# yoseph007/PQA2

Hardware: AMD Instinct MI355X
Metric: VMAF frames/sec (vif+adm+motion2 -> SVM), device-resident synthetic YUV pairs (higher is better)
Workload: dtype f32; 1 GPU; 2160p 3840x2160 8-bit, vmaf_4k_v0.6.1, 300 frames/GPU; frames_per_gpu=300, frames_total=300, batch=97, frames_per_launch=75, clips_pipelined=True, parallelism=frame-shard x1, 1-frame motion halo, all-gather of records + of scores

## Files before the change

### pqa2_amd/csrc/kernels.h

```cpp
#pragma once
#include <hip/hip_runtime.h>
#include <stdint.h>

#include <vector>

namespace pqa {

enum Elem : int { ELEM_U8 = 0, ELEM_U16 = 1, ELEM_F32 = 2 };

struct PlaneRun {
  const void* base;
  int64_t row_pitch;
  int64_t frame_pitch;
};

struct MutPlaneRun {
  void* base;
  int64_t row_pitch;
  int64_t frame_pitch;
};

int vif_tile_w(int scale);
constexpr int kVifTileH = 8;
inline int vif_tiles_x(int scale, int w) { return (w + vif_tile_w(scale) - 1) / vif_tile_w(scale); }
// ... 30 lines not shown
                      float inv_scale, float gain_limit, MutPlaneRun ll_ref, MutPlaneRun ll_dis, double* partials,
                      int* n_partials, hipError_t* err);
bool adm_pyramid_takes(Elem elem, int w, int h);
int adm_pyramid_partials(int w, int h);
bool launch_adm_pyramid(hipStream_t stream, Elem elem, PlaneRun ref, PlaneRun dis, int n_frames, int w, int h, float inv_scale,
                        float gain_limit, MutPlaneRun ll_ref, MutPlaneRun ll_dis, double* partials0, double* partials1,
                        int* n_partials, hipError_t* err);
float adm_dwt_quant_step(int lambda, int theta);

constexpr int kAdmFxRows = kAdmTileH + 2;
struct AdmFxScale {
  int scale, band_w, band_h;
  int left, top, right, bottom;
  float rf[3];
  uint32_t i_rf[3];
  int cm_shift_sq[3], cm_shift_sub[3], cm_shift_cub[3], cm_final_q[3];
  int den_shift_sq, den_shift_cub, den_final_q;
  int num_row_shift, den_row_shift;
};
AdmFxScale adm_fixed_scale_params(int scale, int band_w, int band_h);
void adm_fixed_div_table(int32_t* out65537);
void adm_fixed_epilogue(const AdmFxScale& p, const long long acc[6], double* num_out, double* den_out);
hipError_t launch_adm_fixed(hipStream_t stream, int scale, int bit_depth, Elem elem, PlaneRun ref, PlaneRun dis,
                            int n_frames, int w, int h, double gain_limit, const int32_t* div_lut,
                            MutPlaneRun ll_ref, MutPlaneRun ll_dis, long long* partials);

constexpr int kMotionTileW = 252, kMotionTileH = 16;
inline int motion_tiles(int w, int h) {
  return ((w + kMotionTileW - 1) / kMotionTileW) * ((h + kMotionTileH - 1) / kMotionTileH);
}
enum : int { MOTION_TILED = 0, MOTION_AUTO = 1 };
hipError_t launch_motion(hipStream_t stream, Elem elem, PlaneRun ref, const void* prev0, int64_t prev0_row_pitch,
                         int n_frames, int w, int h, float inv_scale, double* partials, int mode = MOTION_AUTO,
                         int* n_partials = nullptr);
int motion_march_partials(int w, int h);
bool launch_motion_march(hipStream_t stream, Elem elem, PlaneRun ref, const void* prev0, int64_t prev0_row_pitch, int n_frames,
                         int w, int h, double* partials, int* n_partials, hipError_t* err);
hipError_t launch_motion_fixed(hipStream_t stream, int bit_depth, Elem elem, PlaneRun ref, const void* prev0,
                               int64_t prev0_row_pitch, int n_frames, int w, int h, unsigned long long* partials);

constexpr int kSseBlocksPerPlane = 256;
hipError_t launch_sse(hipStream_t stream, Elem elem, PlaneRun a, PlaneRun b, int n_frames, int w, int h,
                      unsigned long long* partials);

constexpr int kSsimTileBW = 32, kSsimTileBH = 8;
inline int ssim_tiles(int w, int h) {
  const int ww = (w >> 2) - 1, wh = (h >> 2) - 1;
  if (ww < 1 || wh < 1) return 0;
  return ((ww + kSsimTileBW - 1) / kSsimTileBW) * ((wh + kSsimTileBH - 1) / kSsimTileBH);
}
hipError_t launch_ssim(hipStream_t stream, Elem elem, PlaneRun main, PlaneRun ref, int n_frames, int w, int h,
                       int max_value, double* partials, unsigned long long* sse_partials);

constexpr int kLumaBlocks = 128;
hipError_t launch_luma_stats(hipStream_t stream, Elem elem, PlaneRun luma, int n_frames, int w, int h,
                             unsigned threshold, int gray_bit_depth, unsigned long long* partials,
                             unsigned long long* out);
void luma_gray_map(int bit_depth, float* a, float* b);

struct FinalizeArgs {
  int n_frames;
  int has_vif, has_adm, has_motion, n_sse_planes, n_ssim_planes;
  const double* vif_part[4];   int vif_tiles[4];
  const long long* vif_fx_part[4];
  const double* adm_part[4];   int adm_tiles[4];   float adm_area[4];
  const long long* adm_fx_part[4];
  int adm_fx_tiles_x[4], adm_fx_top[4], adm_fx_bottom[4], adm_fx_num_shift[4], adm_fx_den_shift[4];
  long long* adm_fx_acc;
  const double* motion_part;   int motion_tiles;   double motion_norm;
  const unsigned long long* motion_fx_part;
// ... 225 lines not shown
```

### pqa2_amd/csrc/motion.hip

```cpp
#include "kernels.h"
#include "pqa_device.h"

namespace pqa {
namespace {

struct MotionArgs {
  const void* ref;
  int64_t row_pitch, frame_pitch;
  const void* prev0;
  int64_t prev0_row_pitch;
  int w, h, tiles_x, n_tiles;
  double* partials;
  f2 vt[6];
  f2 ht[5];
};

constexpr int TW = kMotionTileW, TH = kMotionTileH, R = 2, COLS = TW + 4, NSEG = TW / 4, S = 16, NIN = S + 4;
constexpr int kP2 = 258;
static_assert(COLS <= 256 && NSEG <= 64 && TW % 4 == 0 && TH == S, "one column per thread, one 16-row strip");

template <typename T>
__global__ __launch_bounds__(kBlock) void motion_kernel(const MotionArgs a) {
  __shared__ f2 sv[TH / 2][kP2];
  __shared__ double red[4];
// ... 54 lines not shown
    if (seg < NSEG) {
      f2 in[8];
      const f4* p = reinterpret_cast<const f4*>(&sv[rp][seg * 4]);
#pragma unroll
      for (int q = 0; q < 4; ++q) {
        const f4 v = p[q];
        in[2 * q] = f2{v.x, v.y};
        in[2 * q + 1] = f2{v.z, v.w};
      }
      f2 out[4];
#pragma unroll
      for (int o = 0; o < 4; ++o) out[o] = f2{0.0f, 0.0f};
#pragma unroll
      for (int k = 0; k < 5; ++k)
#pragma unroll
        for (int o = 0; o < 4; ++o) out[o] = __builtin_elementwise_fma(a.ht[k], in[o + k], out[o]);
#pragma unroll
      for (int o = 0; o < 4; ++o) {
        const float mc = (x0 + seg * 4 + o) < a.w ? 1.0f : 0.0f;
        sad = fmaf(mc * mA, fabsf(out[o].x), sad);
        sad = fmaf(mc * mB, fabsf(out[o].y), sad);
      }
    }
  }
  const float part[1] = {sad};
  double v[1];
  block_sum_f32<1>(part, v, red);
  if (tid == 0) a.partials[(int64_t)fr * a.n_tiles + tile] = v[0];
}

}

hipError_t launch_motion(hipStream_t stream, Elem elem, PlaneRun ref, const void* prev0, int64_t prev0_row_pitch,
                         int n_frames, int w, int h, float inv_scale, double* partials, int mode, int* n_partials) {
  if (n_partials) *n_partials = motion_tiles(w, h);
  if (n_frames <= 0) return hipSuccess;
  if (mode == MOTION_AUTO) {
    hipError_t err = hipSuccess;
    if (launch_motion_march(stream, elem, ref, prev0, prev0_row_pitch, n_frames, w, h, partials, n_partials, &err)) return err;
  }
  MotionArgs a{};
  a.ref = ref.base; a.row_pitch = ref.row_pitch; a.frame_pitch = ref.frame_pitch;
  a.prev0 = prev0; a.prev0_row_pitch = prev0_row_pitch;
  a.w = w; a.h = h;
  a.tiles_x = (w + TW - 1) / TW;
  a.n_tiles = motion_tiles(w, h);
  (void)inv_scale;
  a.partials = partials;
  {
    double v[5], sum = 0.0;
    float f[5];
    for (int k = 0; k < 5; ++k) { v[k] = exp(-0.5 * (k - 2) * (k - 2)); sum += v[k]; }
    for (int k = 0; k < 5; ++k) f[k] = (float)(v[k] / sum);
    for (int k = 0; k <= 5; ++k) a.vt[k] = f2{k < 5 ? f[k] : 0.0f, k > 0 ? f[k - 1] : 0.0f};
    for (int k = 0; k < 5; ++k) a.ht[k] = f2{f[k], f[k]};
  }
  const dim3 grid(a.n_tiles, n_frames), block(kBlock);
  switch (elem) {
    case ELEM_U8: hipLaunchKernelGGL((motion_kernel<uint8_t>), grid, block, 0, stream, a); break;
    case ELEM_U16: hipLaunchKernelGGL((motion_kernel<uint16_t>), grid, block, 0, stream, a); break;
    default: return hipErrorInvalidValue;
  }
  return hipGetLastError();
}

}
```

### pqa2_amd/csrc/motion_march.hip

```cpp
#include <cmath>

#include "kernels.h"
#include "pqa_device.h"

namespace pqa {
namespace {

constexpr int kCols = 124;

struct MotionMarchArgs {
  const void* ref;
  unsigned pitch;
  int64_t frame_pitch;
  const void* prev0;
  unsigned prev0_pitch;
  int w, h;
  int aligned, aligned0;
  int n_stripes, n_sg, seg_rows, n_seg;
  float c[5];
  double* partials;
  int n_part;
};

__device__ __forceinline__ float from_left(float v) {
  return __builtin_bit_cast(float, __builtin_amdgcn_update_dpp(0, __builtin_bit_cast(int, v), 0x138, 0xf, 0xf, true));
}
__device__ __forceinline__ float from_right(float v) {
  return __builtin_bit_cast(float, __builtin_amdgcn_update_dpp(0, __builtin_bit_cast(int, v), 0x130, 0xf, 0xf, true));
}

template <typename T, bool EDGE>
struct PairLoader {
  rsrc_t rs;
  unsigned v0, v1, pitch;
  int h;
  struct Raw { unsigned a, b; };
  __device__ __forceinline__ Raw load(int y) const {
    const unsigned so = (unsigned)mirror1(y, h) * pitch;
    if constexpr (EDGE) {
      return Raw{(unsigned)buf_load<T>(rs, v0, so), (unsigned)buf_load<T>(rs, v1, so)};
    } else if constexpr (sizeof(T) == 1) {
      return Raw{(unsigned)(unsigned short)__builtin_amdgcn_raw_buffer_load_b16(rs, v0, so, 0), 0u};
    } else {
      return Raw{(unsigned)__builtin_amdgcn_raw_buffer_load_b32(rs, v0 * 2u, so * 2u, 0), 0u};
    }
  }
  static __device__ __forceinline__ f2 to_float(const Raw r) {
    if constexpr (EDGE) return f2{(float)r.a, (float)r.b};
    else if constexpr (sizeof(T) == 1) return f2{(float)(r.a & 0xffu), (float)((r.a >> 8) & 0xffu)};
    else return f2{(float)(r.a & 0xffffu), (float)(r.a >> 16)};
  }
};

template <typename T, bool EDGE>
__device__ __forceinline__ double march(const MotionMarchArgs& a, const PairLoader<T, EDGE>& cur, const PairLoader<T, EDGE>& prv,
                                        const int r0, const int r1, const int x_first ) {
  const float c0 = a.c[0], c1 = a.c[1], c2 = a.c[2], c3 = a.c[3], c4 = a.c[4];
  f2 p0 = f2{0.0f, 0.0f}, p1 = p0, p2 = p0, p3 = p0;
  float sad0 = 0.0f, sad1 = 0.0f;
  double dsad0 = 0.0, dsad1 = 0.0;
  const int y_end = min(r1, a.h);
  typename PairLoader<T, EDGE>::Raw cs[4], ps[4];
#pragma unroll
  for (int j = 0; j < 4; ++j) { cs[j] = cur.load(r0 - 2 + j); ps[j] = prv.load(r0 - 2 + j); }
  int step = 0;
  for (int y = r0 - 2; y < r1 + 2; y += 4, ++step) {
    f2 d[4];
#pragma unroll
    for (int j = 0; j < 4; ++j) d[j] = PairLoader<T, EDGE>::to_float(cs[j]) - PairLoader<T, EDGE>::to_float(ps[j]);
#pragma unroll
    for (int j = 0; j < 4; ++j) { cs[j] = cur.load(y + 4 + j); ps[j] = prv.load(y + 4 + j); }
    const f2 k0 = f2{c0, c0}, k1 = f2{c1, c1}, k2 = f2{c2, c2}, k3 = f2{c3, c3}, k4 = f2{c4, c4};
    f2 o[4];
    o[0] = __builtin_elementwise_fma(k4, d[0], p0);
    o[1] = __builtin_elementwise_fma(k4, d[1], __builtin_elementwise_fma(k3, d[0], p1));
    o[2] = __builtin_elementwise_fma(k4, d[2], __builtin_elementwise_fma(k3, d[1], __builtin_elementwise_fma(k2, d[0], p2)));
    o[3] = __builtin_elementwise_fma(k4, d[3], __builtin_elementwise_fma(k3, d[2], __builtin_elementwise_fma(k2, d[1], __builtin_elementwise_fma(k1, d[0], p3))));
    p0 = __builtin_elementwise_fma(k3, d[3], __builtin_elementwise_fma(k2, d[2], __builtin_elementwise_fma(k1, d[1], k0 * d[0])));
    p1 = __builtin_elementwise_fma(k2, d[3], __builtin_elementwise_fma(k1, d[2], k0 * d[1]));
    p2 = __builtin_elementwise_fma(k1, d[3], k0 * d[2]);
    p3 = k0 * d[3];
#pragma unroll
    for (int j = 0; j < 4; ++j) {
      const int yo = y - 2 + j;
      const float wrow = __builtin_bit_cast(float, (unsigned)-(int)(yo >= r0 && yo < y_end) & 0x3f800000u);
      const float m0 = o[j].x, m1 = o[j].y;
      const float l0 = from_left(m0), l1 = from_left(m1), q0 = from_right(m0), q1 = from_right(m1);
      const float h0 = fmaf(c4, q0, fmaf(c3, m1, fmaf(c2, m0, fmaf(c1, l1, c0 * l0))));
      const float h1 = fmaf(c4, q1, fmaf(c3, q0, fmaf(c2, m1, fmaf(c1, m0, c0 * l1))));
      sad0 = fmaf(wrow, fabsf(h0), sad0);
      sad1 = fmaf(wrow, fabsf(h1), sad1);
    }
    if ((step & 3) == 3) { dsad0 += (double)sad0; dsad1 += (double)sad1; sad0 = 0.0f; sad1 = 0.0f; }
  }
  dsad0 += (double)sad0;
  dsad1 += (double)sad1;
  const int lane = threadIdx.x & 63;
  const bool own = lane >= 1 && lane <= 62;
  return (own && x_first < a.w ? dsad0 : 0.0) + (own && x_first + 1 < a.w ? dsad1 : 0.0);
}

#ifndef PQA_MOTION_SEG_ROWS
#define PQA_MOTION_SEG_ROWS 128
#endif

template <typename T>
__global__ __launch_bounds__(kBlock) void motion_march_kernel(const MotionMarchArgs a) {
  const int tid = threadIdx.x, lane = tid & 63;
  const int wave = __builtin_amdgcn_readfirstlane(tid >> 6);
  const int id = xcd_remap(blockIdx.x, a.n_sg * a.n_seg);
  const int sg = id % a.n_sg, seg = id / a.n_sg;
  const int stripe = sg * 4 + wave;
  const int fr = blockIdx.y;
  double* __restrict__ part = a.partials + (int64_t)fr * a.n_part + (int64_t)id * 4 + wave;
  const T* __restrict__ cur = (const T*)a.ref + (int64_t)fr * a.frame_pitch;
  const T* __restrict__ prev = fr == 0 ? (const T*)a.prev0 : cur - a.frame_pitch;
  const unsigned pitch_p = fr == 0 ? a.prev0_pitch : a.pitch;
  if (stripe >= a.n_stripes || prev == nullptr) {
    if (lane == 0) *part = 0.0;
    return;
  }
  const int r0 = seg * a.seg_rows, r1 = min(r0 + a.seg_rows, a.h);
  const int cs = stripe * (kCols / 2);
  const int c = cs - 1 + lane;
  const rsrc_t rs_c = make_rsrc(cur, (unsigned)a.h * a.pitch * (unsigned)sizeof(T));
  const rsrc_t rs_p = make_rsrc(prev, (unsigned)a.h * pitch_p * (unsigned)sizeof(T));
  const bool fast = a.aligned && (fr > 0 || a.aligned0) && cs >= 1 && 2 * (cs + kCols / 2) + 1 < a.w;
  double v;
  if (fast) {
    const PairLoader<T, false> lc{rs_c, (unsigned)(2 * c), 0u, a.pitch, a.h}, lp{rs_p, (unsigned)(2 * c), 0u, pitch_p, a.h};
    v = march<T, false>(a, lc, lp, r0, r1, 2 * c);
  } else {
    const unsigned v0 = (unsigned)mirror1(2 * c, a.w), v1 = (unsigned)mirror1(2 * c + 1, a.w);
    const PairLoader<T, true> lc{rs_c, v0, v1, a.pitch, a.h}, lp{rs_p, v0, v1, pitch_p, a.h};
    v = march<T, true>(a, lc, lp, r0, r1, 2 * c);
  }
  v = wave_sum(v);
  if (lane == 0) *part = v;
}

}

int motion_march_partials(int w, int h) {
  const int n_stripes = (w + kCols - 1) / kCols;
  return ((n_stripes + 3) / 4) * 4 * ((h + PQA_MOTION_SEG_ROWS - 1) / PQA_MOTION_SEG_ROWS);
}

bool launch_motion_march(hipStream_t stream, Elem elem, PlaneRun ref, const void* prev0, int64_t prev0_row_pitch, int n_frames,
                         int w, int h, double* partials, int* n_partials, hipError_t* err) {
  if (elem != ELEM_U8 && elem != ELEM_U16) return false;
  const int es = elem == ELEM_U16 ? 2 : 1;
  if ((int64_t)ref.row_pitch * h * es >= (1ll << 31) || (int64_t)prev0_row_pitch * h * es >= (1ll << 31)) return false;
  MotionMarchArgs a{};
  a.ref = ref.base; a.pitch = (unsigned)ref.row_pitch; a.frame_pitch = ref.frame_pitch;
  a.prev0 = prev0; a.prev0_pitch = (unsigned)prev0_row_pitch;
  a.w = w; a.h = h;
  const uintptr_t two = (uintptr_t)(2 * es - 1);
  a.aligned = ((uintptr_t)ref.base & two) == 0 && ((ref.row_pitch | ref.frame_pitch) & 1) == 0;
  a.aligned0 = ((uintptr_t)prev0 & two) == 0 && (prev0_row_pitch & 1) == 0;
  a.n_stripes = (w + kCols - 1) / kCols;
  a.n_sg = (a.n_stripes + 3) / 4;
  a.seg_rows = PQA_MOTION_SEG_ROWS;
  a.n_seg = (h + a.seg_rows - 1) / a.seg_rows;
  {
    double v[5], sum = 0.0;
    for (int k = 0; k < 5; ++k) { v[k] = exp(-0.5 * (k - 2) * (k - 2)); sum += v[k]; }
    for (int k = 0; k < 5; ++k) a.c[k] = (float)(v[k] / sum);
  }
  a.partials = partials;
  a.n_part = a.n_sg * 4 * a.n_seg;
  if (n_partials) *n_partials = a.n_part;
  const dim3 grid(a.n_sg * a.n_seg, n_frames), block(kBlock);
  if (elem == ELEM_U16) hipLaunchKernelGGL((motion_march_kernel<uint16_t>), grid, block, 0, stream, a);
  else hipLaunchKernelGGL((motion_march_kernel<uint8_t>), grid, block, 0, stream, a);
  *err = hipGetLastError();
  return true;
}

}
```

### pqa2_amd/csrc/pqa_api.hip

```cpp
#include "pqa_ctx.h"

#include <algorithm>
#include <cstdarg>
#include <cstdio>
#include <cstdlib>
#include <mutex>

#include "ingest.h"

using namespace pqa;
using pqa::host::PackPool;
using pqa::host::PackTask;
using pqa::host::run_pack_task;

static thread_local std::string g_create_error;

int pqa::fail(pqa_ctx* c, int code, const char* fmt, ...) {
  char buf[512];
  va_list ap;
  va_start(ap, fmt);
  vsnprintf(buf, sizeof buf, fmt, ap);
  va_end(ap);
  if (c) c->err = buf; else g_create_error = buf;
  return code;
// ... 83 lines not shown
                (long long)f, (long long)holder, c->capacity);
  return PQA_OK;
}

void claim_slots(pqa_ctx* c, int64_t first, int n, uint64_t seq) { c->ring.claim(first, n, seq); }

int wait_batch(pqa_ctx* c, uint64_t seq) {
  if (seq <= c->done_seq) return PQA_OK;
  const int e = (int)(seq % kBatchEvents);
  HIPCHK(c, hipEventSynchronize(c->batch_ev[e]));
  c->done_seq = c->batch_ev_seq[e] > seq ? c->batch_ev_seq[e] : seq;
  return PQA_OK;
}

int process_batch(pqa_ctx* c, int64_t first, int n, const pqa_device_clip* ref, const pqa_device_clip* dis,
                  const void* prev, int64_t prev_pitch_bytes) {
  const uint32_t feat = c->cfg.features;
  const int es = c->esize;
  for (int p = 0; p < c->n_planes; ++p) {
    if (ref->row_pitch[p] % es || dis->row_pitch[p] % es || ref->frame_pitch[p] % es || dis->frame_pitch[p] % es)
      return fail(c, PQA_EINVAL, "plane %d pitch is not a multiple of the sample size", p);
    if (!ref->plane[p] || !dis->plane[p]) return fail(c, PQA_EINVAL, "plane %d pointer is null", p);
  }
  {
    const int rc = check_slots_free(c, first, n);
    if (rc != PQA_OK) return rc;
  }
  c->started = true;
  const PlaneRun rY{ref->plane[0], ref->row_pitch[0] / es, ref->frame_pitch[0] / es};
  const PlaneRun dY{dis->plane[0], dis->row_pitch[0] / es, dis->frame_pitch[0] / es};
  const int w = c->pw[0], h = c->ph[0];
  hipStream_t st = c->stream;
  const bool multi = c->multi_stream && !(c->prof && c->prof_mask == 0xffffffffu);
  hipStream_t st_adm = multi ? c->aux[0] : st, st_misc = multi ? c->aux[1] : st;

  const int k = c->k_sub;
  int e0 = 0, sp_n = n;
  if (k > 1) {
    e0 = (int)((k - first % k) % k);
    sp_n = e0 < n ? (n - e0 + k - 1) / k : 0;
  }
  const bool fork_late = multi && c->multi_stream == 2 && (feat & PQA_FEAT_VIF) && !c->vif_fixed && sp_n > 0;
  if (multi && !fork_late) {
    HIPCHK(c, hipEventRecord(c->fork_ev, st));
    HIPCHK(c, hipStreamWaitEvent(st_adm, c->fork_ev, 0));
    HIPCHK(c, hipStreamWaitEvent(st_misc, c->fork_ev, 0));
  }
  const auto sub = [&](PlaneRun r) {
    return PlaneRun{(const uint8_t*)r.base + (int64_t)e0 * r.frame_pitch * es, r.row_pitch, r.frame_pitch * k};
  };
  const PlaneRun rYs = k > 1 ? sub(rY) : rY, dYs = k > 1 ? sub(dY) : dY;

  const void* p0 = prev;
  int64_t p0_pitch = prev_pitch_bytes;
  if (feat & PQA_FEAT_MOTION) {
    if (!p0 && (c->halo_armed || (c->have_last && c->last_index == first - 1))) {
      p0 = c->last_luma;
      p0_pitch = c->last_luma_pitch;
    }
    if (p0 && p0_pitch % es) return fail(c, PQA_EINVAL, "halo pitch is not a multiple of the sample size");
  }
  int vif_np[4] = {c->vif_tiles[0], c->vif_tiles[1], c->vif_tiles[2], c->vif_tiles[3]};
  int adm_np[4] = {c->adm_tiles[0], c->adm_tiles[1], c->adm_tiles[2], c->adm_tiles[3]};
  int motion_np = c->motion_tiles_n;

  if ((feat & PQA_FEAT_VIF) && sp_n > 0 && c->vif_fixed) {
    PlaneRun cr = rYs, cd = dYs;
    Elem ce = c->elem;
    int cw = w, ch = h;
    for (int s = 0; s < 4; ++s) {
      MutPlaneRun nr{nullptr, 0, 0}, nd{nullptr, 0, 0};
      if (s < 3) {
        Level& L = c->vif_lv[s + 1];
        nr = MutPlaneRun{L.ref, L.pitch, L.frame_pitch};
        nd = MutPlaneRun{L.dis, L.pitch, L.frame_pitch};
      }
      {
        ProfScope ps(c, s, sp_n, st);
        HIPCHK(c, launch_vif_fixed(st, s, (int)c->cfg.bit_depth, ce, cr, cd, sp_n, cw, ch, c->cfg.vif_enhn_gain_limit,
                                   c->vif_lut, c->vif_fx_part[s], nr, nd));
      }
      if (s < 3) {
        Level& L = c->vif_lv[s + 1];
        cr = PlaneRun{L.ref, L.pitch, L.frame_pitch};
        cd = PlaneRun{L.dis, L.pitch, L.frame_pitch};
        ce = ELEM_U16;
        cw = L.w; ch = L.h;
      }
    }
  } else if ((feat & PQA_FEAT_VIF) && sp_n > 0) {
    PlaneRun cr = rYs, cd = dYs;
    Elem ce = c->elem;
    int cw = w, ch = h;
    for (int s = 0; s < 4; ++s) {
      MutPlaneRun nr{nullptr, 0, 0}, nd{nullptr, 0, 0};
      if (s < 3) {
        Level& L = c->vif_lv[s + 1];
        nr = MutPlaneRun{L.ref, L.pitch, L.frame_pitch};
        nd = MutPlaneRun{L.dis, L.pitch, L.frame_pitch};
      }
      {
        ProfScope ps(c, s, sp_n, st);
        HIPCHK(c, launch_vif_stat(st, s, ce, cr, cd, sp_n, cw, ch, c->inv_scale,
                                  (float)c->cfg.vif_enhn_gain_limit, c->cfg.vif_border == PQA_VIF_BORDER_INTEGER,
                                  c->vif_part[s], nr, nd, c->vif_s0_mode, &vif_np[s], c->vif_uniform));
      }
      if (s == 0 && fork_late) {
        HIPCHK(c, hipEventRecord(c->fork_ev, st));
        HIPCHK(c, hipStreamWaitEvent(st_adm, c->fork_ev, 0));
        HIPCHK(c, hipStreamWaitEvent(st_misc, c->fork_ev, 0));
      }
      if (s < 3) {
        Level& L = c->vif_lv[s + 1];
        cr = PlaneRun{L.ref, L.pitch, L.frame_pitch};
        cd = PlaneRun{L.dis, L.pitch, L.frame_pitch};
        ce = ELEM_F32;
        cw = L.w; ch = L.h;
      }
    }
  }
  if ((feat & PQA_FEAT_ADM) && sp_n > 0 && c->adm_fixed) {
    PlaneRun cr = rYs, cd = dYs;
    Elem ce = c->elem;
    int cw = w, ch = h;
    for (int s = 0; s < 4; ++s) {
      MutPlaneRun lr{nullptr, 0, 0}, ld{nullptr, 0, 0};
      if (s < 3) {
        Level& L = c->adm_lv[s + 1];
        lr = MutPlaneRun{L.ref, L.pitch, L.frame_pitch};
        ld = MutPlaneRun{L.dis, L.pitch, L.frame_pitch};
      }
      {
        ProfScope ps(c, 7 + s, sp_n, st_adm);
        HIPCHK(c, launch_adm_fixed(st_adm, s, (int)c->cfg.bit_depth, ce, cr, cd, sp_n, cw, ch,
                                   c->cfg.adm_enhn_gain_limit, c->adm_div_lut, lr, ld, c->adm_fx_part[s]));
      }
      if (s < 3) {
        Level& L = c->adm_lv[s + 1];
        cr = PlaneRun{L.ref, L.pitch, L.frame_pitch};
        cd = PlaneRun{L.dis, L.pitch, L.frame_pitch};
        ce = ELEM_F32;
        cw = L.w; ch = L.h;
      }
// ... 11 lines not shown
      if (launch_adm_pyramid(st_adm, ce, cr, cd, sp_n, cw, ch, c->inv_scale, (float)c->cfg.adm_enhn_gain_limit,
                             MutPlaneRun{L2.ref, L2.pitch, L2.frame_pitch}, MutPlaneRun{L2.dis, L2.pitch, L2.frame_pitch},
                             c->adm_part[0], c->adm_part[1], &np, &perr)) {
        HIPCHK(c, perr);
        adm_np[0] = adm_np[1] = np;
        cr = PlaneRun{L2.ref, L2.pitch, L2.frame_pitch};
        cd = PlaneRun{L2.dis, L2.pitch, L2.frame_pitch};
        ce = ELEM_F32;
        cw = L2.w; ch = L2.h;
        s = 2;
      }
    }
    for (; s < 4; ++s) {
      MutPlaneRun lr{nullptr, 0, 0}, ld{nullptr, 0, 0};
      if (s < 3) {
        Level& L = c->adm_lv[s + 1];
        lr = MutPlaneRun{L.ref, L.pitch, L.frame_pitch};
        ld = MutPlaneRun{L.dis, L.pitch, L.frame_pitch};
      }
      {
        ProfScope ps(c, 7 + s, sp_n, st_adm);
        HIPCHK(c, launch_adm_scale(st_adm, s, ce, cr, cd, sp_n, cw, ch, c->inv_scale,
                                   (float)c->cfg.adm_enhn_gain_limit, lr, ld, c->adm_part[s], c->adm_mode, &adm_np[s]));
      }
      if (s < 3) {
        Level& L = c->adm_lv[s + 1];
        cr = PlaneRun{L.ref, L.pitch, L.frame_pitch};
        cd = PlaneRun{L.dis, L.pitch, L.frame_pitch};
        ce = ELEM_F32;
        cw = L.w; ch = L.h;
      }
    }
  }
  if (feat & PQA_FEAT_MOTION) {
    ProfScope ps(c, 11, n, st_misc);
    if (c->motion_fixed)
      HIPCHK(c, launch_motion_fixed(st_misc, (int)c->cfg.bit_depth, c->elem, rY, p0, p0 ? p0_pitch / es : 0, n, w, h,
                                    c->motion_fx_part));
    else
      HIPCHK(c, launch_motion(st_misc, c->elem, rY, p0, p0 ? p0_pitch / es : 0, n, w, h, c->inv_scale, c->motion_part,
                              c->motion_mode, &motion_np));
  }
  int n_sse = 0, n_ssim = 0;
  bool sse_a[3] = {false, false, false}, sse_b[3] = {false, false, false}, sse_t[3] = {false, false, false};
  const bool both = (feat & PQA_FEAT_PSNR) && (feat & PQA_FEAT_SSIM);
  if (feat & PQA_FEAT_PSNR) {
    n_sse = c->n_planes;
    ProfScope ps(c, 12, n, st_misc);
    for (int p = 0; p < c->n_planes; ++p) {
      const PlaneRun a{dis->plane[p], dis->row_pitch[p] / es, dis->frame_pitch[p] / es};
      const PlaneRun b{ref->plane[p], ref->row_pitch[p] / es, ref->frame_pitch[p] / es};
      const int pw = c->pw[p], ph = c->ph[p];
      if (both && c->ssim_tiles_n[p] > 0) {
        sse_t[p] = true;
        const int w4 = (pw >> 2) << 2, h4 = (ph >> 2) << 2;
        if (w4 < pw) {
          const PlaneRun ar{(const uint8_t*)a.base + (int64_t)w4 * es, a.row_pitch, a.frame_pitch};
          const PlaneRun br{(const uint8_t*)b.base + (int64_t)w4 * es, b.row_pitch, b.frame_pitch};
          HIPCHK(c, launch_sse(st_misc, c->elem, ar, br, n, pw - w4, ph, c->sse_part[p]));
          sse_a[p] = true;
        }
        if (h4 < ph) {
          const PlaneRun ab{(const uint8_t*)a.base + (int64_t)h4 * a.row_pitch * es, a.row_pitch, a.frame_pitch};
          const PlaneRun bb{(const uint8_t*)b.base + (int64_t)h4 * b.row_pitch * es, b.row_pitch, b.frame_pitch};
          HIPCHK(c, launch_sse(st_misc, c->elem, ab, bb, n, w4, ph - h4, c->sse_part_b[p]));
          sse_b[p] = true;
        }
      } else {
        HIPCHK(c, launch_sse(st_misc, c->elem, a, b, n, pw, ph, c->sse_part[p]));
        sse_a[p] = true;
      }
    }
  }
  if (feat & PQA_FEAT_SSIM) {
// ... 178 lines not shown
        spp[z] = c->st_hist_pitch / es;
      }
    }
    if (prev) {
      if (prev_pitch_bytes % es) return fail(c, PQA_EINVAL, "halo pitch is not a multiple of the sample size");
      sp0[1] = prev;
      spp[1] = prev_pitch_bytes / es;
    }
    const PlaneRun sc[2] = {dY, rY};
    const bool sfull[2] = {(feat & PQA_FEAT_SITI_DIS_FULL) != 0, (feat & PQA_FEAT_SITI_REF_FULL) != 0};
    HIPCHK(c, launch_siti(st_misc, c->elem, sc, sp0, spp, sfull, 2, n, w, h, c->st_part, c->ext4, PQA_EXT4_DOUBLES,
                          (int)(first % c->capacity), c->capacity, nullptr));
  }
  if (feat & PQA_FEAT_INTEGRITY) {
    if (c->ig_armed) {
      c->ig_hist_idx = first - 1;
      c->ig_armed = false;
    }
    const bool have = c->ig_hist_idx >= 0 && c->ig_hist_idx == first - 1;
    PlaneRun cur[3] = {};
    const void* ip0[3] = {nullptr, nullptr, nullptr};
    int64_t ipp[3] = {0, 0, 0};
    for (int p = 0; p < c->n_planes; ++p) {
      cur[p] = PlaneRun{dis->plane[p], dis->row_pitch[p] / es, dis->frame_pitch[p] / es};
      if (have) {
        ip0[p] = c->ig_hist[p];
        ipp[p] = c->ig_hist_pitch[p] / es;
      }
    }
    HIPCHK(c, launch_integrity(st_misc, c->elem, cur, ip0, ipp, c->pw, c->ph, c->n_planes, n, false, c->black_thr,
                               c->ig_part, c->ext5, PQA_EXT5_DOUBLES, (int)(first % c->capacity), c->capacity, nullptr));
  }

  if (multi) {
    HIPCHK(c, hipEventRecord(c->join_ev[0], st_adm));
    HIPCHK(c, hipEventRecord(c->join_ev[1], st_misc));
    HIPCHK(c, hipStreamWaitEvent(st, c->join_ev[0], 0));
    HIPCHK(c, hipStreamWaitEvent(st, c->join_ev[1], 0));
  }

  FinalizeArgs fa{};
  for (int s = 0; s < 4; ++s) {
    fa.vif_part[s] = c->vif_part[s]; fa.vif_tiles[s] = c->vif_fixed ? c->vif_tiles[s] : vif_np[s];
    fa.vif_fx_part[s] = c->vif_fixed ? c->vif_fx_part[s] : nullptr;
    fa.adm_part[s] = c->adm_part[s]; fa.adm_tiles[s] = c->adm_fixed ? c->adm_tiles[s] : adm_np[s]; fa.adm_area[s] = c->adm_area[s];
    fa.adm_fx_part[s] = c->adm_fixed ? c->adm_fx_part[s] : nullptr;
    fa.adm_fx_tiles_x[s] = adm_tiles_x(c->adm_fx[s].band_w);
    fa.adm_fx_top[s] = c->adm_fx[s].top; fa.adm_fx_bottom[s] = c->adm_fx[s].bottom;
    fa.adm_fx_num_shift[s] = c->adm_fx[s].num_row_shift; fa.adm_fx_den_shift[s] = c->adm_fx[s].den_row_shift;
  }
  fa.motion_part = c->motion_part;
  fa.motion_tiles = c->motion_fixed ? c->motion_tiles_n : motion_np;
  fa.motion_norm = (double)c->inv_scale / ((double)w * h);
  fa.motion_fx_part = c->motion_fixed ? c->motion_fx_part : nullptr;
  fa.motion_wh = (unsigned)w * (unsigned)h;
  for (int p = 0; p < 3; ++p) {
    fa.sse_part[p] = c->sse_part[p];
    fa.sse_use_a[p] = sse_a[p] ? 1 : 0;
    fa.sse_part_b[p] = sse_b[p] ? c->sse_part_b[p] : nullptr;
    fa.sse_tile_part[p] = sse_t[p] ? c->sse_tile_part[p] : nullptr;
    fa.ssim_part[p] = c->ssim_part[p]; fa.ssim_tiles[p] = c->ssim_tiles_n[p]; fa.ssim_norm[p] = c->ssim_norm[p];
  }
  fa.adm_fx_acc = c->adm_fx_acc;
  fa.records = c->records;
  fa.record_stride = PQA_RECORD_DOUBLES;
  fa.capacity = c->capacity;
  {
    ProfScope ps(c, 14, n, st);
    if (k > 1) {
      if (sp_n > 0 && (feat & (PQA_FEAT_VIF | PQA_FEAT_ADM))) {
// ... 380 lines not shown
  }
  if (c->B > 256) c->B = 256;
  c->HB = c->B < 8 ? c->B : 8;
  c->capacity = cfg->result_capacity ? (int)cfg->result_capacity : 16384;
  if (c->capacity < c->B) c->capacity = c->B;
  c->k_sub = cfg->n_subsample > 1 ? (int)cfg->n_subsample : 1;
  if (c->cfg.vif_enhn_gain_limit <= 0) c->cfg.vif_enhn_gain_limit = 100.0;
  if (c->cfg.adm_enhn_gain_limit <= 0) c->cfg.adm_enhn_gain_limit = 100.0;
  c->elem = cfg->bit_depth > 8 ? ELEM_U16 : ELEM_U8;
  c->esize = cfg->bit_depth > 8 ? 2 : 1;
  c->inv_scale = 1.0f / (float)(1 << (cfg->bit_depth - 8));
  c->n_planes = (int)cfg->n_planes;
  c->pw[0] = (int)cfg->width; c->ph[0] = (int)cfg->height;
  for (int p = 1; p < 3; ++p) {
    c->pw[p] = (int)((cfg->width + (1u << cfg->chroma_hshift) - 1) >> cfg->chroma_hshift);
    c->ph[p] = (int)((cfg->height + (1u << cfg->chroma_vshift) - 1) >> cfg->chroma_vshift);
  }

  auto bail = [&](int rc) {
    g_create_error = c->err;
    pqa_destroy(c);
    return rc;
  };
#define CREATE_TRY(expr) do { int rc_ = (expr); if (rc_ != PQA_OK) return bail(rc_); } while (0)
#define CREATE_HIP(expr) do { hipError_t e_ = (expr); if (e_ != hipSuccess) { \
    fail(c, e_ == hipErrorOutOfMemory ? PQA_ENOMEM : PQA_EDEVICE, "%s failed: %s", #expr, hipGetErrorString(e_)); \
    return bail(e_ == hipErrorOutOfMemory ? PQA_ENOMEM : PQA_EDEVICE); } } while (0)

  CREATE_HIP(hipSetDevice(c->device));
  CREATE_HIP(hipStreamCreateWithFlags(&c->own_stream, hipStreamNonBlocking));
  c->stream = c->own_stream;
  {
    const char* e = getenv("PQA_MULTI_STREAM");
    c->multi_stream = (e && e[0] == '1') ? 1 : (e && e[0] == '2') ? 2 : 0;
    const char* t = getenv("PQA_TRACE");
    c->trace = t && t[0] == '1';
    const char* v = getenv("PQA_VIF_MFMA");
    c->vif_s0_mode = (v && v[0] == '0') ? VIF_S0_VALU : VIF_S0_AUTO;
    const char* vu = getenv("PQA_VIF_UNIFORM");
    c->vif_uniform = !(vu && vu[0] == '0');
    const char* am = getenv("PQA_ADM_MARCH");
    const char* ap = getenv("PQA_ADM_PYRAMID");
    c->adm_mode = (am && am[0] == '0') ? ADM_TILED : (ap && ap[0] == '0') ? ADM_MARCH : ADM_AUTO;
    const char* mm = getenv("PQA_MOTION_MARCH");
    c->motion_mode = (mm && mm[0] == '0') ? MOTION_TILED : MOTION_AUTO;
    const char* xm = getenv("PQA_XSSE_MFMA");
    c->xsse_mfma = !(xm && xm[0] == '0');
  }
  for (int i = 0; i < 2; ++i) {
    CREATE_HIP(hipStreamCreateWithFlags(&c->aux[i], hipStreamNonBlocking));
    CREATE_HIP(hipEventCreateWithFlags(&c->join_ev[i], hipEventDisableTiming));
  }
  CREATE_HIP(hipEventCreateWithFlags(&c->fork_ev, hipEventDisableTiming));
  for (int i = 0; i < kBatchEvents; ++i) CREATE_HIP(hipEventCreateWithFlags(&c->batch_ev[i], hipEventDisableTiming));
  try {
    c->ring.init(c->capacity);
  } catch (...) {
    fail(c, PQA_ENOMEM, "out of host memory");
    return bail(PQA_ENOMEM);
  }

  c->vif_fixed = (cfg->features & PQA_FEAT_VIF) && (cfg->fixed_point & PQA_FIXED_VIF);
  c->motion_fixed = (cfg->features & PQA_FEAT_MOTION) && (cfg->fixed_point & PQA_FIXED_MOTION);
  c->adm_fixed = (cfg->features & PQA_FEAT_ADM) && (cfg->fixed_point & PQA_FIXED_ADM);
  if (c->adm_fixed) {
    std::vector<int32_t> lut(65537);
    adm_fixed_div_table(lut.data());
// ... 716 lines not shown
```

### pqa2_amd/csrc/pqa_ctx.h

```cpp
#pragma once
#include "../../include/pqa_vmaf.h"

#include <atomic>
#include <cstring>
#include <memory>
#include <string>
#include <thread>
#include <vector>

#include "host_pack.h"
#include "host_ring.h"
#include "kernels.h"

namespace pqa {

struct Level {
  int w = 0, h = 0;
  int64_t pitch = 0, frame_pitch = 0;
  float* ref = nullptr;
  float* dis = nullptr;
};

struct Half {
  uint8_t* pinned = nullptr;
// ... 122 lines not shown
  bool xsse_mfma = true;
  pqa::RsCached rs_cache[pqa::kRsCached];
  int rs_next = 0;
  uint8_t* rs_pin[2] = {nullptr, nullptr};
  size_t rs_pin_cap[2] = {0, 0};
  void* side_buf[pqa::kSideBufs] = {};
  size_t side_cap[pqa::kSideBufs] = {};
  uint8_t* last_luma = nullptr;
  int64_t last_luma_pitch = 0;
  int64_t last_index = -1;
  bool have_last = false, halo_armed = false;
  pqa::Half half[2];
  int cur_half = 0, pending = 0;
  int64_t pending_first = 0;
  size_t slot_bytes = 0;
  size_t plane_off[2][3] = {};
  int64_t slot_row_pitch[3] = {};
  bool staging_ready = false;
  std::thread pin_thread;
  hipError_t pin_err = hipSuccess;
  uint8_t* surf_dev = nullptr;
  std::unique_ptr<pqa::host::PackPool> pack_pool;
  bool pack_pool_tried = false;
  std::vector<pqa::host::PackTask> pack_tasks;
  pqa::host::RecordRing ring;
  hipEvent_t batch_ev[pqa::kBatchEvents] = {};
  uint64_t batch_ev_seq[pqa::kBatchEvents] = {};
  uint64_t batch_seq = 0;
  uint64_t done_seq = 0;
  std::atomic<int> cancelled{0};
  std::string err;
  std::vector<void*> allocs;
  int multi_stream = 0;
  int vif_s0_mode = pqa::VIF_S0_AUTO;
  int vif_uniform = 1;
  int adm_mode = pqa::ADM_AUTO;
  int motion_mode = pqa::MOTION_AUTO;
  bool trace = false;
  bool prof = false;
  uint32_t prof_mask = 0xffffffffu;
  std::vector<pqa::ProfEv> evs;
  double prof_ms[PQA_PROF_KERNELS] = {};
  uint64_t prof_n[PQA_PROF_KERNELS] = {}, prof_frames[PQA_PROF_KERNELS] = {};
};

namespace pqa {

int fail(pqa_ctx* c, int code, const char* fmt, ...);

#define HIPCHK(c, expr)                                                                          \
  do {                                                                                           \
    hipError_t e_ = (expr);                                                                      \
    if (e_ != hipSuccess)                                                                        \
      return pqa::fail((c), e_ == hipErrorOutOfMemory ? PQA_ENOMEM : PQA_EDEVICE, "%s failed: %s", #expr, \
                  hipGetErrorString(e_));                                                        \
  } while (0)

template <typename T>
int dev_alloc(pqa_ctx* c, T** out, size_t count) {
  void* p = nullptr;
  if (count == 0) count = 1;
  HIPCHK(c, hipMalloc(&p, count * sizeof(T)));
  c->allocs.push_back(p);
  *out = (T*)p;
  return PQA_OK;
}
// ... 13 lines not shown
```

Before: 22260 frames/s.

## Add DPP horizontal taps in motion march, single-wave variant, and motion guest stream

Replaces the cross-lane shuffles plus FMAs of the motion march horizontal 5-tap filter with inline-asm DPP multiply/FMA instructions that read neighbour lanes directly. This path is on by default for non-edge tiles. The change also adds an optional one-wave-per-block launch variant with a min-blocks launch bound, and a 'guest' multi-stream mode (3/4) that runs motion alone on an aux stream early, overlapping it with VIF and ADM. The stream and wave options are opt-in through environment variables. The DPP asm relies on wave_shr/wave_shl semantics with bound_ctrl and hand-placed s_nop hazards, so it risks miscompiled or incorrect edge lanes.

```diff
diff --git a/pqa2_amd/csrc/kernels.h b/pqa2_amd/csrc/kernels.h
--- a/pqa2_amd/csrc/kernels.h
+++ b/pqa2_amd/csrc/kernels.h
@@ -86,10 +86,10 @@
 enum : int { MOTION_TILED = 0, MOTION_AUTO = 1 };
 hipError_t launch_motion(hipStream_t stream, Elem elem, PlaneRun ref, const void* prev0, int64_t prev0_row_pitch,
                          int n_frames, int w, int h, float inv_scale, double* partials, int mode = MOTION_AUTO,
-                         int* n_partials = nullptr);
+                         int* n_partials = nullptr, int march_waves = 4);
 int motion_march_partials(int w, int h);
 bool launch_motion_march(hipStream_t stream, Elem elem, PlaneRun ref, const void* prev0, int64_t prev0_row_pitch, int n_frames,
-                         int w, int h, double* partials, int* n_partials, hipError_t* err);
+                         int w, int h, double* partials, int* n_partials, hipError_t* err, int waves = 4);
 hipError_t launch_motion_fixed(hipStream_t stream, int bit_depth, Elem elem, PlaneRun ref, const void* prev0,
                                int64_t prev0_row_pitch, int n_frames, int w, int h, unsigned long long* partials);
 
diff --git a/pqa2_amd/csrc/motion.hip b/pqa2_amd/csrc/motion.hip
--- a/pqa2_amd/csrc/motion.hip
+++ b/pqa2_amd/csrc/motion.hip
@@ -110,12 +110,13 @@
 }
 
 hipError_t launch_motion(hipStream_t stream, Elem elem, PlaneRun ref, const void* prev0, int64_t prev0_row_pitch,
-                         int n_frames, int w, int h, float inv_scale, double* partials, int mode, int* n_partials) {
+                         int n_frames, int w, int h, float inv_scale, double* partials, int mode, int* n_partials,
+                         int march_waves) {
   if (n_partials) *n_partials = motion_tiles(w, h);
   if (n_frames <= 0) return hipSuccess;
   if (mode == MOTION_AUTO) {
     hipError_t err = hipSuccess;
-    if (launch_motion_march(stream, elem, ref, prev0, prev0_row_pitch, n_frames, w, h, partials, n_partials, &err)) return err;
+    if (launch_motion_march(stream, elem, ref, prev0, prev0_row_pitch, n_frames, w, h, partials, n_partials, &err, march_waves)) return err;
   }
   MotionArgs a{};
   a.ref = ref.base; a.row_pitch = ref.row_pitch; a.frame_pitch = ref.frame_pitch;
diff --git a/pqa2_amd/csrc/motion_march.hip b/pqa2_amd/csrc/motion_march.hip
--- a/pqa2_amd/csrc/motion_march.hip
+++ b/pqa2_amd/csrc/motion_march.hip
@@ -7,6 +7,10 @@
 namespace {
 
 constexpr int kCols = 124;
+
+#ifndef PQA_MOTION_DPP_TAPS
+#define PQA_MOTION_DPP_TAPS 1
+#endif
 
 struct MotionMarchArgs {
   const void* ref;
@@ -56,6 +60,9 @@
 __device__ __forceinline__ double march(const MotionMarchArgs& a, const PairLoader<T, EDGE>& cur, const PairLoader<T, EDGE>& prv,
                                         const int r0, const int r1, const int x_first ) {
   const float c0 = a.c[0], c1 = a.c[1], c2 = a.c[2], c3 = a.c[3], c4 = a.c[4];
+  constexpr bool kDpp = PQA_MOTION_DPP_TAPS && !EDGE;
+  float t0 = c0, t1 = c1, t3 = c3, t4 = c4;
+  if constexpr (kDpp) asm volatile("" : "+v"(t0), "+v"(t1), "+v"(t3), "+v"(t4));
   f2 p0 = f2{0.0f, 0.0f}, p1 = p0, p2 = p0, p3 = p0;
   float sad0 = 0.0f, sad1 = 0.0f;
   double dsad0 = 0.0, dsad1 = 0.0;
@@ -85,9 +92,26 @@
       const int yo = y - 2 + j;
       const float wrow = __builtin_bit_cast(float, (unsigned)-(int)(yo >= r0 && yo < y_end) & 0x3f800000u);
       const float m0 = o[j].x, m1 = o[j].y;
-      const float l0 = from_left(m0), l1 = from_left(m1), q0 = from_right(m0), q1 = from_right(m1);
-      const float h0 = fmaf(c4, q0, fmaf(c3, m1, fmaf(c2, m0, fmaf(c1, l1, c0 * l0))));
-      const float h1 = fmaf(c4, q1, fmaf(c3, q0, fmaf(c2, m1, fmaf(c1, m0, c0 * l1))));
+      float h0, h1;
+      if constexpr (kDpp) {
+        asm("s_nop 1\n\t"
+            "v_mul_f32_dpp %0, %2, %4 wave_shr:1 row_mask:0xf bank_mask:0xf bound_ctrl:1\n\t"
+            "v_mul_f32_dpp %1, %3, %4 wave_shr:1 row_mask:0xf bank_mask:0xf bound_ctrl:1\n\t"
+            "v_fmac_f32_dpp %0, %3, %5 wave_shr:1 row_mask:0xf bank_mask:0xf bound_ctrl:1\n\t"
+            "v_fmac_f32_e32 %1, %8, %2\n\t"
+            "v_fmac_f32_e32 %0, %9, %2\n\t"
+            "v_fmac_f32_e32 %1, %9, %3\n\t"
+            "v_fmac_f32_e32 %0, %10, %3\n\t"
+            "v_fmac_f32_dpp %1, %2, %6 wave_shl:1 row_mask:0xf bank_mask:0xf bound_ctrl:1\n\t"
+            "v_fmac_f32_dpp %0, %2, %7 wave_shl:1 row_mask:0xf bank_mask:0xf bound_ctrl:1\n\t"
+            "v_fmac_f32_dpp %1, %3, %7 wave_shl:1 row_mask:0xf bank_mask:0xf bound_ctrl:1"
+            : "=&v"(h0), "=&v"(h1)
+            : "v"(m0), "v"(m1), "v"(t0), "v"(t1), "v"(t3), "v"(t4), "s"(c1), "s"(c2), "s"(c3));
+      } else {
+        const float l0 = from_left(m0), l1 = from_left(m1), q0 = from_right(m0), q1 = from_right(m1);
+        h0 = fmaf(c4, q0, fmaf(c3, m1, fmaf(c2, m0, fmaf(c1, l1, c0 * l0))));
+        h1 = fmaf(c4, q1, fmaf(c3, q0, fmaf(c2, m1, fmaf(c1, m0, c0 * l1))));
+      }
       sad0 = fmaf(wrow, fabsf(h0), sad0);
       sad1 = fmaf(wrow, fabsf(h1), sad1);
     }
@@ -104,11 +128,18 @@
 #define PQA_MOTION_SEG_ROWS 128
 #endif
 
-template <typename T>
-__global__ __launch_bounds__(kBlock) void motion_march_kernel(const MotionMarchArgs a) {
+template <typename T, int WAVES>
+__global__ __launch_bounds__(64 * WAVES, 8) void motion_march_kernel(const MotionMarchArgs a) {
   const int tid = threadIdx.x, lane = tid & 63;
-  const int wave = __builtin_amdgcn_readfirstlane(tid >> 6);
-  const int id = xcd_remap(blockIdx.x, a.n_sg * a.n_seg);
+  int wave, id;
+  if constexpr (WAVES == 4) {
+    wave = __builtin_amdgcn_readfirstlane(tid >> 6);
+    id = xcd_remap(blockIdx.x, a.n_sg * a.n_seg);
+  } else {
+    const int g = xcd_remap(blockIdx.x, a.n_sg * a.n_seg * 4);
+    wave = g & 3;
+    id = g >> 2;
+  }
   const int sg = id % a.n_sg, seg = id / a.n_sg;
   const int stripe = sg * 4 + wave;
   const int fr = blockIdx.y;
@@ -147,7 +178,7 @@
 }
 
 bool launch_motion_march(hipStream_t stream, Elem elem, PlaneRun ref, const void* prev0, int64_t prev0_row_pitch, int n_frames,
-                         int w, int h, double* partials, int* n_partials, hipError_t* err) {
+                         int w, int h, double* partials, int* n_partials, hipError_t* err, int waves) {
   if (elem != ELEM_U8 && elem != ELEM_U16) return false;
   const int es = elem == ELEM_U16 ? 2 : 1;
   if ((int64_t)ref.row_pitch * h * es >= (1ll << 31) || (int64_t)prev0_row_pitch * h * es >= (1ll << 31)) return false;
@@ -170,9 +201,15 @@
   a.partials = partials;
   a.n_part = a.n_sg * 4 * a.n_seg;
   if (n_partials) *n_partials = a.n_part;
-  const dim3 grid(a.n_sg * a.n_seg, n_frames), block(kBlock);
-  if (elem == ELEM_U16) hipLaunchKernelGGL((motion_march_kernel<uint16_t>), grid, block, 0, stream, a);
-  else hipLaunchKernelGGL((motion_march_kernel<uint8_t>), grid, block, 0, stream, a);
+  if (waves == 1) {
+    const dim3 grid(a.n_sg * a.n_seg * 4, n_frames), block(64);
+    if (elem == ELEM_U16) hipLaunchKernelGGL((motion_march_kernel<uint16_t, 1>), grid, block, 0, stream, a);
+    else hipLaunchKernelGGL((motion_march_kernel<uint8_t, 1>), grid, block, 0, stream, a);
+  } else {
+    const dim3 grid(a.n_sg * a.n_seg, n_frames), block(kBlock);
+    if (elem == ELEM_U16) hipLaunchKernelGGL((motion_march_kernel<uint16_t, 4>), grid, block, 0, stream, a);
+    else hipLaunchKernelGGL((motion_march_kernel<uint8_t, 4>), grid, block, 0, stream, a);
+  }
   *err = hipGetLastError();
   return true;
 }
diff --git a/pqa2_amd/csrc/pqa_api.hip b/pqa2_amd/csrc/pqa_api.hip
--- a/pqa2_amd/csrc/pqa_api.hip
+++ b/pqa2_amd/csrc/pqa_api.hip
@@ -139,7 +139,9 @@
   const int w = c->pw[0], h = c->ph[0];
   hipStream_t st = c->stream;
   const bool multi = c->multi_stream && !(c->prof && c->prof_mask == 0xffffffffu);
-  hipStream_t st_adm = multi ? c->aux[0] : st, st_misc = multi ? c->aux[1] : st;
+  const bool guest = multi && c->multi_stream >= 3;
+  hipStream_t st_adm = multi && !guest ? c->aux[0] : st, st_misc = multi && !guest ? c->aux[1] : st;
+  hipStream_t st_motion = guest ? c->aux[1] : st_misc;
 
   const int k = c->k_sub;
   int e0 = 0, sp_n = n;
@@ -147,11 +149,17 @@
     e0 = (int)((k - first % k) % k);
     sp_n = e0 < n ? (n - e0 + k - 1) / k : 0;
   }
-  const bool fork_late = multi && c->multi_stream == 2 && (feat & PQA_FEAT_VIF) && !c->vif_fixed && sp_n > 0;
+  const bool fork_late = multi && (c->multi_stream == 2 || c->multi_stream == 4) && (feat & PQA_FEAT_VIF) && !c->vif_fixed && sp_n > 0;
+  const auto fork = [&]() -> int {
+    HIPCHK(c, hipEventRecord(c->fork_ev, st));
+    if (st_adm != st) HIPCHK(c, hipStreamWaitEvent(st_adm, c->fork_ev, 0));
+    if (st_misc != st) HIPCHK(c, hipStreamWaitEvent(st_misc, c->fork_ev, 0));
+    if (st_motion != st && st_motion != st_misc) HIPCHK(c, hipStreamWaitEvent(st_motion, c->fork_ev, 0));
+    return PQA_OK;
+  };
   if (multi && !fork_late) {
-    HIPCHK(c, hipEventRecord(c->fork_ev, st));
-    HIPCHK(c, hipStreamWaitEvent(st_adm, c->fork_ev, 0));
-    HIPCHK(c, hipStreamWaitEvent(st_misc, c->fork_ev, 0));
+    const int rc = fork();
+    if (rc != PQA_OK) return rc;
   }
   const auto sub = [&](PlaneRun r) {
     return PlaneRun{(const uint8_t*)r.base + (int64_t)e0 * r.frame_pitch * es, r.row_pitch, r.frame_pitch * k};
@@ -171,6 +179,21 @@
   int adm_np[4] = {c->adm_tiles[0], c->adm_tiles[1], c->adm_tiles[2], c->adm_tiles[3]};
   int motion_np = c->motion_tiles_n;
 
+  const auto motion_chain = [&]() -> int {
+    if (!(feat & PQA_FEAT_MOTION)) return PQA_OK;
+    ProfScope ps(c, 11, n, st_motion);
+    if (c->motion_fixed)
+      HIPCHK(c, launch_motion_fixed(st_motion, (int)c->cfg.bit_depth, c->elem, rY, p0, p0 ? p0_pitch / es : 0, n, w, h,
+                                    c->motion_fx_part));
+    else
+      HIPCHK(c, launch_motion(st_motion, c->elem, rY, p0, p0 ? p0_pitch / es : 0, n, w, h, c->inv_scale, c->motion_part,
+                              c->motion_mode, &motion_np, c->motion_waves));
+    return PQA_OK;
+  };
+  if (guest && !fork_late) {
+    const int rc = motion_chain();
+    if (rc != PQA_OK) return rc;
+  }
   if ((feat & PQA_FEAT_VIF) && sp_n > 0 && c->vif_fixed) {
     PlaneRun cr = rYs, cd = dYs;
     Elem ce = c->elem;
@@ -213,9 +236,9 @@
                                   c->vif_part[s], nr, nd, c->vif_s0_mode, &vif_np[s], c->vif_uniform));
       }
       if (s == 0 && fork_late) {
-        HIPCHK(c, hipEventRecord(c->fork_ev, st));
-        HIPCHK(c, hipStreamWaitEvent(st_adm, c->fork_ev, 0));
-        HIPCHK(c, hipStreamWaitEvent(st_misc, c->fork_ev, 0));
+        int rc = fork();
+        if (rc == PQA_OK && guest) rc = motion_chain();
+        if (rc != PQA_OK) return rc;
       }
       if (s < 3) {
         Level& L = c->vif_lv[s + 1];
@@ -293,14 +316,9 @@
       }
     }
   }
-  if (feat & PQA_FEAT_MOTION) {
-    ProfScope ps(c, 11, n, st_misc);
-    if (c->motion_fixed)
-      HIPCHK(c, launch_motion_fixed(st_misc, (int)c->cfg.bit_depth, c->elem, rY, p0, p0 ? p0_pitch / es : 0, n, w, h,
-                                    c->motion_fx_part));
-    else
-      HIPCHK(c, launch_motion(st_misc, c->elem, rY, p0, p0 ? p0_pitch / es : 0, n, w, h, c->inv_scale, c->motion_part,
-                              c->motion_mode, &motion_np));
+  if (!guest) {
+    const int rc = motion_chain();
+    if (rc != PQA_OK) return rc;
   }
   int n_sse = 0, n_ssim = 0;
   bool sse_a[3] = {false, false, false}, sse_b[3] = {false, false, false}, sse_t[3] = {false, false, false};
@@ -545,10 +563,13 @@
                                c->ig_part, c->ext5, PQA_EXT5_DOUBLES, (int)(first % c->capacity), c->capacity, nullptr));
   }
 
-  if (multi) {
+  if (multi && !guest) {
     HIPCHK(c, hipEventRecord(c->join_ev[0], st_adm));
     HIPCHK(c, hipEventRecord(c->join_ev[1], st_misc));
     HIPCHK(c, hipStreamWaitEvent(st, c->join_ev[0], 0));
+    HIPCHK(c, hipStreamWaitEvent(st, c->join_ev[1], 0));
+  } else if (guest) {
+    HIPCHK(c, hipEventRecord(c->join_ev[1], st_motion));
     HIPCHK(c, hipStreamWaitEvent(st, c->join_ev[1], 0));
   }
 
@@ -995,7 +1016,9 @@
   c->stream = c->own_stream;
   {
     const char* e = getenv("PQA_MULTI_STREAM");
-    c->multi_stream = (e && e[0] == '1') ? 1 : (e && e[0] == '2') ? 2 : 0;
+    c->multi_stream = (e && e[0] >= '1' && e[0] <= '4' && !e[1]) ? e[0] - '0' : 0;
+    const char* mw = getenv("PQA_MOTION_WAVES");
+    c->motion_waves = (mw && mw[0] == '1' && !mw[1]) ? 1 : 4;
     const char* t = getenv("PQA_TRACE");
     c->trace = t && t[0] == '1';
     const char* v = getenv("PQA_VIF_MFMA");
diff --git a/pqa2_amd/csrc/pqa_ctx.h b/pqa2_amd/csrc/pqa_ctx.h
--- a/pqa2_amd/csrc/pqa_ctx.h
+++ b/pqa2_amd/csrc/pqa_ctx.h
@@ -178,6 +178,7 @@
   std::string err;
   std::vector<void*> allocs;
   int multi_stream = 0;
+  int motion_waves = 4;
   int vif_s0_mode = pqa::VIF_S0_AUTO;
   int vif_uniform = 1;
   int adm_mode = pqa::ADM_AUTO;
```

After: 21900 frames/s. -1.6%, worse.
